# nianticlabs/mickey

Hardware: NVIDIA H100
Metric: image-pairs/sec @720x540 (higher is better)
Workload: dtype f16 operands / f32 accumulate (tensor core), f32 matcher+solver

## Files before the change

include/mickey_b200.h:

```cpp
#ifndef MICKEY_B200_H
#define MICKEY_B200_H

#ifdef __cplusplus
extern "C" {
#endif

typedef struct mk_handle mk_handle;

typedef struct mk_config {
  int embed_dim, depth, heads;
  int down_factor;
  int block_dims[4];
  int desc_dim;
  int use_softmax;
  int depth_sigmoid;
  float max_depth;
  int kp_pos_enc, dsc_pos_enc;
  int norm_dsc;
  float temperature;
  int use_dustbin;
  int it_matches, it_ransac;
  int num_sampled, num_corr, num_refine;
  float th_inlier, th_soft_inlier;
} mk_config;
// ... 111 lines not shown
#define MK_RB_GRAD_W2 4
#define MK_RB_GRAD_WSC 8
#define MK_RB_GRAD_BN1_W 16
#define MK_RB_GRAD_BN1_B 32
#define MK_RB_GRAD_BN2_W 64
#define MK_RB_GRAD_BN2_B 128
typedef struct mk_resblock_params {
  const float* w1; const float* w2; const float* wsc;
  const float* bn1_w; const float* bn1_b; float* bn1_mean; float* bn1_var;
  const float* bn2_w; const float* bn2_b; float* bn2_mean; float* bn2_var;
  float eps1, eps2, momentum1, momentum2;
} mk_resblock_params;
typedef struct mk_resblock_grads {
  float* dx; float* w1; float* w2; float* wsc; float* bn1_w; float* bn1_b; float* bn2_w; float* bn2_b;
} mk_resblock_grads;
long long mk_resblock_ws_bytes(int B, int h, int w, int cin, int cout);
long long mk_resblock_saved_bytes(int B, int h, int w, int cin, int cout);
long long mk_resblock_backward_ws_bytes(int B, int h, int w, int cin, int cout);
int mk_resblock_forward(const float* x_dev, const long long* x_strides_host, int B, int h, int w, int cin, int cout,
                        const mk_resblock_params* params_host, int flags, float* out_dev, void* saved_dev,
                        long long saved_bytes, void* ws_dev, long long ws_bytes, void* stream);
int mk_resblock_backward(const void* saved_dev, const float* grad_out_dev, const long long* g_strides_host,
                         const float* out_dev, int B, int h, int w, int cin, int cout, const mk_resblock_params* params_host,
                         int flags, int want, const mk_resblock_grads* grads_host, void* ws_dev, long long ws_bytes,
                         void* stream);

#define MK_HO_SCORE_SOFTMAX 0
#define MK_HO_SCORE_SIGMOID 1
#define MK_HO_OFFSET 2
#define MK_HO_DEPTH 3
#define MK_HO_DEPTH_SIGMOID 4
#define MK_HO_DESC_L2 5
long long mk_head_out_backward_ws_bytes(int kind, int B, int h, int w, int C);
int mk_head_out_forward(int kind, const float* x_dev, const long long* x_strides_host, int B, int C, int h, int w,
                        const float* weight_dev, const float* eps_dev, float temperature, float max_depth, float* out_dev,
                        float* norm_dev, void* stream);
int mk_head_out_backward(int kind, const float* x_dev, const long long* x_strides_host, int B, int C, int h, int w,
                         const float* weight_dev, float temperature, float max_depth, const float* out_dev,
                         const float* norm_dev, const float* grad_out_dev, float* grad_x_dev, float* grad_w_dev, void* ws_dev,
                         long long ws_bytes, void* stream);

int mk_set_seed(mk_handle* h, unsigned long long seed, void* stream);

long long mk_launch_count(mk_handle* h);
int mk_pdl_enabled(void);
int mk_profile_enable(mk_handle* h, int enable);
int mk_profile_read(mk_handle* h, char* buf, int buf_bytes);

typedef struct mk_gemm_args {
  int epi;
  int impl;
  const void* a; long long a_rows, a_cols, a_ld;
  const void* b; long long b_rows, b_cols, b_ld;
  int M, N, k_chunks, chunks_per_tap, num_taps;
  int tap_shift[9];
  int groups, a_row_group_off, a_col_group_off, a_col_base, b_row_group_off;
  int act;
  const float* bias; int bias_group_off;
  const float* gamma; const float* beta; int ln_group_off;
  float* out_f; long long out_f_ld, out_f_group_off;
  void* out_h; long long out_h_ld, out_h_group_off;
  const void* res_h; long long res_h_ld, res_h_group_off;
  const float* aux; int aux_group_mask;
  int pad_h2, pad_w2, tok_per_img;
  float eps;
  int n_valid; float inv_temp;
  const float* dustbin;
  float* part_row; float* part_col; int part_ld;
  const float* lse_r; const float* lse_c;
  const float* scr0; const float* scr1;
  float* scores; float* kp_scores; float* final_scores;
  float lse_bound;
  long long out_pitch;
} mk_gemm_args;

int mk_op_gemm(const mk_gemm_args* args, void* stream);
int mk_op_patch_gather(const float* img, void* patches_h, int n_img, int H, int W, int kpad, float* x_f,
                       const float* cls_pos, int D, void* stream);
int mk_op_ingest_u8(const unsigned char* img_u8, void* patches_h, int n_img, int H, int W, int kpad, float* x_f,
                    const float* cls_pos, int D, void* stream);
int mk_op_layernorm(const float* x, const float* w, const float* b, void* out_h, int rows, int D, float eps, int mode,
                    int gh, int gw, void* stream);
int mk_op_attention(const void* qkv_h, void* out_h, int n_img, int T, int D, int heads, int impl, void* stream);
int mk_op_linattn(const float* qkv_f, float* kv_part_f, float* kv_f, void* msg_h, int n_img, int G, int h2, int w2, float eps,
                  void* stream);
int mk_op_matcher_reduce(const float* part_row, const float* part_col, const float* dustbin, int B, int N, int part_ld,
                         float* lse_r, float* lse_c, void* stream);
int mk_op_sample(const float* final_scores, int B, int N, long long pitch, int IM, int n_sample, unsigned long long seed, void* ws,
                 long long ws_bytes, int* idx_out, int* status, void* stream);
long long mk_op_sample_workspace_bytes(int B, int IM);
int mk_op_kabsch(const double* H, double* R, int n, void* stream);

int mk_resblock_layout(int B, int h, int w, int cin, int cout, long long* saved_off, long long* bwd_off);
long long mk_op_conv_tf32_ws_bytes(int mode, int B, int h, int w, int cin, int cout, int taps);
int mk_op_conv_tf32(int mode, const float* a, const float* b, float* out, int B, int h, int w, int cin, int cout, int taps,
                    void* ws, long long ws_bytes, void* stream);

#ifdef __cplusplus
}
#endif
#endif
```

mickey_b200/_lib.py:

```python
from __future__ import annotations

import ctypes as C
import math
import os

import torch

_HERE = os.path.dirname(os.path.abspath(__file__))
LIB_PATH = os.path.join(_HERE, "_C", "libmickey_b200.so")


class MkConfig(C.Structure):
    _fields_ = [
        ("embed_dim", C.c_int), ("depth", C.c_int), ("heads", C.c_int),
        ("down_factor", C.c_int),
        ("block_dims", C.c_int * 4),
        ("desc_dim", C.c_int),
        ("use_softmax", C.c_int), ("depth_sigmoid", C.c_int), ("max_depth", C.c_float),
        ("kp_pos_enc", C.c_int), ("dsc_pos_enc", C.c_int), ("norm_dsc", C.c_int),
        ("temperature", C.c_float), ("use_dustbin", C.c_int),
        ("it_matches", C.c_int), ("it_ransac", C.c_int),
        ("num_sampled", C.c_int), ("num_corr", C.c_int), ("num_refine", C.c_int),
        ("th_inlier", C.c_float), ("th_soft_inlier", C.c_float),
    ]
# ... 63 lines not shown
    "mk_extract_images": (C.c_int, [C.c_void_p, C.c_void_p, C.c_int, C.c_int, C.c_int, C.c_void_p, C.c_void_p, C.c_void_p,
                                    C.c_void_p, C.c_void_p, C.c_longlong, C.c_void_p]),
    "mk_extract_images_u8": (C.c_int, [C.c_void_p, C.c_void_p, C.c_int, C.c_int, C.c_int, C.c_void_p, C.c_void_p, C.c_void_p,
                                       C.c_void_p, C.c_void_p, C.c_longlong, C.c_void_p]),
    "mk_forward_pairs": (C.c_int, [C.c_void_p, C.c_void_p, C.c_void_p, C.c_void_p, C.c_void_p, C.c_int,
                                   C.c_void_p, C.c_void_p, C.c_void_p, C.c_void_p, C.c_int,
                                   C.c_void_p, C.c_void_p, C.c_void_p, C.c_void_p, C.c_int, C.c_ulonglong,
                                   C.c_void_p, C.c_void_p, C.c_void_p, C.c_void_p, C.c_void_p, C.c_longlong,
                                   C.c_void_p, C.c_void_p, C.c_void_p, C.c_void_p, C.c_void_p, C.c_void_p, C.c_longlong,
                                   C.c_void_p]),
    "mk_backbone_ws_bytes": (C.c_longlong, [C.c_void_p, C.c_int, C.c_int, C.c_int]),
    "mk_backbone_features": (C.c_int, [C.c_void_p, C.c_void_p, C.c_int, C.c_int, C.c_int, C.c_void_p, C.c_void_p,
                                       C.c_longlong, C.c_void_p]),
    "mk_match": (C.c_int, [C.c_void_p, C.c_int, C.c_void_p, C.c_void_p, C.c_void_p, C.c_longlong, C.c_void_p, C.c_longlong, C.c_void_p]),
    "mk_solve_pose": (C.c_int, [C.c_void_p, C.c_void_p, C.c_longlong, C.c_void_p, C.c_void_p, C.c_void_p, C.c_void_p, C.c_int, C.c_int,
                                C.c_ulonglong, C.c_void_p, C.c_void_p, C.c_void_p, C.c_void_p, C.c_void_p, C.c_void_p,
                                C.c_void_p, C.c_void_p, C.c_void_p, C.c_longlong, C.c_void_p]),
    "mk_forward": (C.c_int, [C.c_void_p, C.c_void_p, C.c_void_p, C.c_void_p, C.c_int, C.c_int, C.c_int, C.c_ulonglong,
                             C.c_void_p, C.c_void_p, C.c_void_p, C.c_void_p, C.c_void_p, C.c_void_p, C.c_void_p, C.c_longlong,
                             C.c_void_p, C.c_void_p, C.c_void_p, C.c_void_p, C.c_void_p, C.c_void_p, C.c_longlong,
                             C.c_void_p]),
    "mk_forward_u8": (C.c_int, [C.c_void_p, C.c_void_p, C.c_void_p, C.c_void_p, C.c_int, C.c_int, C.c_int, C.c_ulonglong,
                                C.c_void_p, C.c_void_p, C.c_void_p, C.c_void_p, C.c_void_p, C.c_void_p, C.c_void_p, C.c_longlong,
                                C.c_void_p, C.c_void_p, C.c_void_p, C.c_void_p, C.c_void_p, C.c_void_p, C.c_longlong,
                                C.c_void_p]),
    "mk_mutual_matches": (C.c_int, [C.c_void_p, C.c_longlong, C.c_int, C.c_int, C.c_float, C.c_void_p, C.c_void_p,
                                    C.c_void_p, C.c_void_p, C.c_longlong, C.c_void_p]),
    "mk_mutual_matches_ws_bytes": (C.c_longlong, [C.c_int, C.c_int]),
    "mk_loss_search": (C.c_int, [C.c_void_p, C.c_longlong, C.c_void_p, C.c_void_p, C.c_void_p, C.c_void_p, C.c_void_p,
                                 C.c_void_p, C.c_int, C.c_int, C.c_int, C.c_int, C.c_int, C.c_int, C.c_int, C.c_float,
                                 C.c_ulonglong, C.c_void_p, C.c_void_p, C.c_void_p, C.c_void_p, C.c_void_p, C.c_void_p,
                                 C.c_void_p, C.c_longlong, C.c_void_p]),
    "mk_loss_search_ws_bytes": (C.c_longlong, [C.c_int, C.c_int]),
    "mk_loss_gradient": (C.c_int, [C.c_void_p, C.c_void_p, C.c_void_p, C.c_void_p, C.c_int, C.c_int, C.c_int, C.c_int,
                                   C.c_void_p, C.c_void_p, C.c_longlong, C.c_void_p]),
    "mk_loss_gradient_ws_bytes": (C.c_longlong, [C.c_int, C.c_int, C.c_int]),
    "mk_dual_softmax_ws_bytes": (C.c_longlong, [C.c_int, C.c_int]),
    "mk_dual_softmax_backward_ws_bytes": (C.c_longlong, [C.c_int, C.c_int]),
    "mk_dual_softmax": (C.c_int, [C.c_void_p, C.c_void_p, C.c_void_p, C.c_void_p, C.c_void_p, C.c_float, C.c_int, C.c_int,
                                  C.c_int, C.c_void_p, C.c_void_p, C.c_void_p, C.c_longlong, C.c_void_p, C.c_void_p,
                                  C.c_void_p, C.c_longlong, C.c_void_p]),
    "mk_dual_softmax_backward": (C.c_int, [C.c_void_p, C.c_void_p, C.c_void_p, C.c_void_p, C.c_void_p, C.c_float, C.c_int,
                                           C.c_int, C.c_void_p, C.c_void_p, C.c_void_p, C.c_longlong, C.c_void_p,
                                           C.c_longlong, C.c_void_p, C.c_longlong, C.c_void_p, C.c_void_p, C.c_void_p,
                                           C.c_void_p, C.c_void_p, C.c_void_p, C.c_longlong, C.c_void_p]),
    "mk_head_transformer_ws_bytes": (C.c_longlong, [C.c_int, C.c_int, C.c_int, C.c_int, C.c_int]),
    "mk_head_transformer_backward_ws_bytes": (C.c_longlong, [C.c_int, C.c_int, C.c_int, C.c_int]),
    "mk_head_transformer": (C.c_int, [C.c_void_p, C.c_void_p, C.c_int, C.c_int, C.c_int, C.POINTER(MkHtrLayer), C.c_int,
                                      C.c_void_p, C.c_int, C.c_void_p, C.c_longlong, C.c_void_p]),
    "mk_head_transformer_backward": (C.c_int, [C.c_void_p, C.c_void_p, C.c_int, C.c_int, C.c_int, C.POINTER(MkHtrLayer),
                                               C.c_int, C.c_void_p, C.POINTER(MkHtrLayerGrads), C.c_void_p, C.c_longlong,
                                               C.c_void_p]),
    "mk_resblock_ws_bytes": (C.c_longlong, [C.c_int, C.c_int, C.c_int, C.c_int, C.c_int]),
    "mk_resblock_saved_bytes": (C.c_longlong, [C.c_int, C.c_int, C.c_int, C.c_int, C.c_int]),
    "mk_resblock_backward_ws_bytes": (C.c_longlong, [C.c_int, C.c_int, C.c_int, C.c_int, C.c_int]),
    "mk_resblock_forward": (C.c_int, [C.c_void_p, C.POINTER(C.c_longlong), C.c_int, C.c_int, C.c_int, C.c_int, C.c_int,
                                      C.POINTER(MkResblockParams), C.c_int, C.c_void_p, C.c_void_p, C.c_longlong,
                                      C.c_void_p, C.c_longlong, C.c_void_p]),
    "mk_resblock_layout": (C.c_int, [C.c_int, C.c_int, C.c_int, C.c_int, C.c_int, C.POINTER(C.c_longlong),
                                     C.POINTER(C.c_longlong)]),
    "mk_resblock_backward": (C.c_int, [C.c_void_p, C.c_void_p, C.POINTER(C.c_longlong), C.c_void_p, C.c_int, C.c_int,
                                       C.c_int, C.c_int, C.c_int, C.POINTER(MkResblockParams), C.c_int, C.c_int,
                                       C.POINTER(MkResblockGrads), C.c_void_p, C.c_longlong, C.c_void_p]),
    "mk_head_out_backward_ws_bytes": (C.c_longlong, [C.c_int, C.c_int, C.c_int, C.c_int, C.c_int]),
    "mk_head_out_forward": (C.c_int, [C.c_int, C.c_void_p, C.POINTER(C.c_longlong), C.c_int, C.c_int, C.c_int, C.c_int,
                                      C.c_void_p, C.c_void_p, C.c_float, C.c_float, C.c_void_p, C.c_void_p, C.c_void_p]),
    "mk_head_out_backward": (C.c_int, [C.c_int, C.c_void_p, C.POINTER(C.c_longlong), C.c_int, C.c_int, C.c_int, C.c_int,
                                       C.c_void_p, C.c_float, C.c_float, C.c_void_p, C.c_void_p, C.c_void_p, C.c_void_p,
                                       C.c_void_p, C.c_void_p, C.c_longlong, C.c_void_p]),
    "mk_pose_to_submission": (C.c_int, [C.c_void_p, C.c_int, C.c_void_p, C.c_void_p]),
    "mk_launch_count": (C.c_longlong, [C.c_void_p]),
    "mk_pdl_enabled": (C.c_int, []),
    "mk_set_seed": (C.c_int, [C.c_void_p, C.c_ulonglong, C.c_void_p]),
    "mk_profile_enable": (C.c_int, [C.c_void_p, C.c_int]),
    "mk_profile_read": (C.c_int, [C.c_void_p, C.c_char_p, C.c_int]),
    "mk_op_gemm": (C.c_int, [C.POINTER(MkGemmArgs), C.c_void_p]),
    "mk_op_patch_gather": (C.c_int, [C.c_void_p, C.c_void_p, C.c_int, C.c_int, C.c_int, C.c_int, C.c_void_p, C.c_void_p,
                                     C.c_int, C.c_void_p]),
    "mk_op_ingest_u8": (C.c_int, [C.c_void_p, C.c_void_p, C.c_int, C.c_int, C.c_int, C.c_int, C.c_void_p, C.c_void_p,
                                  C.c_int, C.c_void_p]),
    "mk_op_layernorm": (C.c_int, [C.c_void_p, C.c_void_p, C.c_void_p, C.c_void_p, C.c_int, C.c_int, C.c_float, C.c_int,
                                  C.c_int, C.c_int, C.c_void_p]),
    "mk_op_attention": (C.c_int, [C.c_void_p, C.c_void_p, C.c_int, C.c_int, C.c_int, C.c_int, C.c_int, C.c_void_p]),
    "mk_op_linattn": (C.c_int, [C.c_void_p, C.c_void_p, C.c_void_p, C.c_void_p, C.c_int, C.c_int, C.c_int, C.c_int, C.c_float, C.c_void_p]),
    "mk_op_matcher_reduce": (C.c_int, [C.c_void_p, C.c_void_p, C.c_void_p, C.c_int, C.c_int, C.c_int, C.c_void_p, C.c_void_p, C.c_void_p]),
    "mk_op_sample": (C.c_int, [C.c_void_p, C.c_int, C.c_int, C.c_longlong, C.c_int, C.c_int, C.c_ulonglong, C.c_void_p, C.c_longlong,
                               C.c_void_p, C.c_void_p, C.c_void_p]),
    "mk_op_sample_workspace_bytes": (C.c_longlong, [C.c_int, C.c_int]),
    "mk_op_kabsch": (C.c_int, [C.c_void_p, C.c_void_p, C.c_int, C.c_void_p]),
    "mk_op_conv_tf32_ws_bytes": (C.c_longlong, [C.c_int, C.c_int, C.c_int, C.c_int, C.c_int, C.c_int, C.c_int]),
    "mk_op_conv_tf32": (C.c_int, [C.c_int, C.c_void_p, C.c_void_p, C.c_void_p, C.c_int, C.c_int, C.c_int, C.c_int, C.c_int,
                                  C.c_int, C.c_void_p, C.c_longlong, C.c_void_p]),
}

STRUCTS = {"mk_config": MkConfig, "mk_gemm_args": MkGemmArgs, "mk_htr_layer": MkHtrLayer,
           "mk_htr_layer_grads": MkHtrLayerGrads, "mk_resblock_params": MkResblockParams,
           "mk_resblock_grads": MkResblockGrads}

_lib = None


class MickeyB200Error(RuntimeError):
    pass


def load():
    global _lib
    if _lib is not None:
        return _lib
    if not os.path.exists(LIB_PATH):
        raise MickeyB200Error(
            f"{LIB_PATH} not found. Build it with `python -m mickey_b200.build` (needs nvcc; sm_90a only). "
            "mickey_b200 has no CPU or PyTorch fallback.")
    lib = C.CDLL(LIB_PATH)
    for name, (res, args) in EXPORTS.items():
        fn = getattr(lib, name)
        fn.restype = res
        fn.argtypes = args
    sizes = {name: (lib.mk_sizeof(name.encode()), C.sizeof(st)) for name, st in STRUCTS.items()}
    bad = [f"{name} {lib_size} vs {py_size}" for name, (lib_size, py_size) in sizes.items() if lib_size != py_size]
    if bad:
        raise MickeyB200Error("ctypes struct layout does not match the library (stale build?): " + ", ".join(bad))
    _lib = lib
    return lib


def check(rc: int, what: str = ""):
    if rc != 0:
        msg = load().mk_last_error().decode(errors="replace")
        raise MickeyB200Error(f"{what} failed (code {rc}): {msg}")


def ptr(t):
    return None if t is None else C.c_void_p(t.data_ptr())


def stream(dev=None):
    return C.c_void_p(torch.cuda.current_stream(dev).cuda_stream)


def workspace(nbytes, dev, what: str):
    nbytes = int(nbytes)
    if nbytes < 0:
        raise MickeyB200Error(f"{what} returned {nbytes}: {load().mk_last_error().decode(errors='replace')}")
    return torch.empty(max(nbytes, 1), dtype=torch.uint8, device=dev)


def pitched(t):
    B, N, _ = t.shape
    s0, s1, s2 = t.stride()
    if s2 == 1 and s1 >= N and (B == 1 or s0 == N * s1):
        return t, s1
    return t.contiguous(), N


class Handle:

    def __init__(self, device, cfg: MkConfig):
        self.lib = load()
        self.device = device
        h = C.c_void_p()
        check(self.lib.mk_create(device.index or 0, C.byref(cfg), C.byref(h)), "mk_create")
        self.h = h

    def __del__(self):
        try:
# ... 17 lines not shown
```

mickey_b200/csrc/attention_tc.cu:

```cuda
#include "gemm_tc.cuh"
#include "ops.h"
#include "gemm.h"
#include <algorithm>
#include <cstdlib>
#include <cstring>

namespace mk {

constexpr int FA_BQ = 192, FA_BK = 128, FA_D = 64, FA_KV_STAGES = 4;
constexpr int FA_CONSUMERS = 3, FA_THREADS = 128 * (FA_CONSUMERS + 1), FA_WARP_TMA = 4 * FA_CONSUMERS;
constexpr int FA_REGS_PRODUCER = 32, FA_REGS_CONSUMER = 160;
static_assert(FA_REGS_PRODUCER * 128 + FA_REGS_CONSUMER * 128 * FA_CONSUMERS <= 65536, "attention: register budget");
constexpr int FA_Q_BYTES = FA_BQ * 128;
constexpr int FA_KV_BYTES = FA_BK * 128;
constexpr int FA_O_BYTES = 64 * 128;
constexpr int FA_REGION = 2 * FA_Q_BYTES + 2 * FA_KV_STAGES * FA_KV_BYTES + FA_CONSUMERS * FA_O_BYTES;
constexpr int FA_SMEM = FA_REGION + 1024 + 256;
static_assert(FA_SMEM <= 227 * 1024, "attention: shared memory");

__device__ __forceinline__ float ex2_approx(float x) {
  float y;
  asm("ex2.approx.ftz.f32 %0, %1;" : "=f"(y) : "f"(x));
  return y;
}

__device__ __forceinline__ void wgmma_m64n64k16_rs_tb(float (&d)[32], const uint32_t (&a)[4], uint64_t desc_b) {
  asm volatile(
      "{\n\t.reg .pred p;\n\tsetp.ne.b32 p, %37, 0;\n\t"
      "wgmma.mma_async.sync.aligned.m64n64k16.f32.f16.f16 "
      "{%0, %1, %2, %3, %4, %5, %6, %7, %8, %9, %10, %11, %12, %13, %14, %15, %16, %17, %18, %19, %20, %21, %22, %23, %24, %25, %26, %27, %28, %29, %30, %31}, {%32, %33, %34, %35}, %36, p, 1, 1, 1;\n\t}"
      : "+f"(d[0]), "+f"(d[1]), "+f"(d[2]), "+f"(d[3]), "+f"(d[4]), "+f"(d[5]), "+f"(d[6]), "+f"(d[7]), "+f"(d[8]), "+f"(d[9]), "+f"(d[10]), "+f"(d[11]), "+f"(d[12]), "+f"(d[13]), "+f"(d[14]), "+f"(d[15]), "+f"(d[16]), "+f"(d[17]), "+f"(d[18]), "+f"(d[19]), "+f"(d[20]), "+f"(d[21]), "+f"(d[22]), "+f"(d[23]), "+f"(d[24]), "+f"(d[25]), "+f"(d[26]), "+f"(d[27]), "+f"(d[28]), "+f"(d[29]), "+f"(d[30]), "+f"(d[31])
      : "r"(a[0]), "r"(a[1]), "r"(a[2]), "r"(a[3]), "l"(desc_b), "r"(1u));
}

__device__ __forceinline__ void warpgroup_sync(int wg) { asm volatile("bar.sync %0, 128;" ::"r"(2 + wg) : "memory"); }

struct AttnTile { int qt, head, im; };
__device__ __forceinline__ AttnTile attn_tile(int t, int q_tiles, int heads) {
  const int bh = t / q_tiles;
  return {t - bh * q_tiles, bh % heads, bh / heads};
}

__device__ __forceinline__ void softmax_tile(float (&s)[64], uint32_t (&p)[8][4], float (&m_run)[2], float (&l_run)[2],
                                             float (&alpha)[2], float scale_log2, int valid, int lane) {
  if (valid < FA_BK) {
#pragma unroll
    for (int i = 0; i < 64; ++i) {
      const int col = 8 * (i >> 2) + 2 * (lane & 3) + (i & 1);
      if (col >= valid) s[i] = -INFINITY;
    }
  }
#pragma unroll
  for (int h = 0; h < 2; ++h) {
    float mx = -INFINITY;
#pragma unroll
    for (int c = 0; c < 16; ++c) mx = fmaxf(mx, fmaxf(s[4 * c + 2 * h], s[4 * c + 2 * h + 1]));
    mx = fmaxf(mx, __shfl_xor_sync(0xffffffffu, mx, 1));
    mx = fmaxf(mx, __shfl_xor_sync(0xffffffffu, mx, 2));
    const float m_new = fmaxf(m_run[h], mx * scale_log2);
    alpha[h] = ex2_approx(m_run[h] - m_new);
    m_run[h] = m_new;
    float sum = 0.f;
#pragma unroll
    for (int c = 0; c < 16; ++c) {
      const float p0 = ex2_approx(fmaf(s[4 * c + 2 * h], scale_log2, -m_new));
      const float p1 = ex2_approx(fmaf(s[4 * c + 2 * h + 1], scale_log2, -m_new));
      const __half2 ph = __floats2half2_rn(p0, p1);
      const float2 r = __half22float2(ph);
      p[c >> 1][2 * (c & 1) + h] = *reinterpret_cast<const uint32_t*>(&ph);
      sum += r.x + r.y;
    }
    l_run[h] = l_run[h] * alpha[h] + sum;
  }
}

__global__ void __launch_bounds__(FA_THREADS, 1)
attention_tc_kernel(const __grid_constant__ CUtensorMap tmQ, const __grid_constant__ CUtensorMap tmKV,
                    const __grid_constant__ CUtensorMap tmO, int T, int heads, int q_tiles, int n_tiles_total, float scale_log2) {
  extern __shared__ uint8_t smem_raw[];
  const uint32_t raw = smem_u32(smem_raw);
  const uint32_t base = (raw + 1023u) & ~1023u;
  const uint32_t sQ = base;
  const uint32_t sK = sQ + 2 * FA_Q_BYTES;
  const uint32_t sV = sK + FA_KV_STAGES * FA_KV_BYTES;
  const uint32_t sO = sV + FA_KV_STAGES * FA_KV_BYTES;
  const uint32_t bars = base + FA_REGION;
  const uint32_t k_full = bars, k_empty = k_full + 8 * FA_KV_STAGES, v_full = k_empty + 8 * FA_KV_STAGES,
                 v_empty = v_full + 8 * FA_KV_STAGES, q_full = v_empty + 8 * FA_KV_STAGES, q_empty = q_full + 16;

  const int warp = threadIdx.x >> 5, lane = threadIdx.x & 31;
  const int D = heads * FA_D;
  const int n_kv = (T + FA_BK - 1) / FA_BK;

  if (warp == FA_WARP_TMA && lane == 0) {
    asm volatile("prefetch.tensormap [%0];" ::"l"(&tmQ) : "memory");
    asm volatile("prefetch.tensormap [%0];" ::"l"(&tmKV) : "memory");
    asm volatile("prefetch.tensormap [%0];" ::"l"(&tmO) : "memory");
    for (int s = 0; s < FA_KV_STAGES; ++s) {
      mbar_init(k_full + 8 * s, 1); mbar_init(k_empty + 8 * s, 4 * FA_CONSUMERS);
      mbar_init(v_full + 8 * s, 1); mbar_init(v_empty + 8 * s, 4 * FA_CONSUMERS);
    }
    for (int b = 0; b < 2; ++b) { mbar_init(q_full + 8 * b, 1); mbar_init(q_empty + 8 * b, 4 * FA_CONSUMERS); }
    asm volatile("fence.mbarrier_init.release.cluster;" ::: "memory");
  }
  __syncthreads();
  pdl_wait();

  if (warp >= FA_WARP_TMA) {
    setmaxnreg_dec<FA_REGS_PRODUCER>();
    if (warp == FA_WARP_TMA && elect_one()) {
      int st = 0;
      uint32_t ph = 0;
      int it = 0;
      for (int t = blockIdx.x; t < n_tiles_total; t += gridDim.x, ++it) {
        const AttnTile tile = attn_tile(t, q_tiles, heads);
        const int row_base = tile.im * T;
        const int qb = it & 1;
        mbar_wait(q_empty + 8 * qb, ((it >> 1) & 1) ^ 1);
        mbar_expect_tx(q_full + 8 * qb, FA_Q_BYTES);
        tma_load_2d(sQ + qb * FA_Q_BYTES, &tmQ, q_full + 8 * qb, tile.head * FA_D, row_base + tile.qt * FA_BQ);
        for (int j = 0; j < n_kv; ++j) {
          mbar_wait(k_empty + 8 * st, ph ^ 1);
          mbar_expect_tx(k_full + 8 * st, FA_KV_BYTES);
          tma_load_2d(sK + st * FA_KV_BYTES, &tmKV, k_full + 8 * st, D + tile.head * FA_D, row_base + j * FA_BK);
          mbar_wait(v_empty + 8 * st, ph ^ 1);
          mbar_expect_tx(v_full + 8 * st, FA_KV_BYTES);
          tma_load_2d(sV + st * FA_KV_BYTES, &tmKV, v_full + 8 * st, 2 * D + tile.head * FA_D, row_base + j * FA_BK);
          if (++st == FA_KV_STAGES) { st = 0; ph ^= 1; }
        }
      }
    }
    __syncwarp();
    pdl_trigger();
    return;
  }

  setmaxnreg_inc<FA_REGS_CONSUMER>();
  const int wg = warp >> 2;
  const uint32_t stage_o = sO + wg * FA_O_BYTES;
  int ks = 0, vs = 0;
  uint32_t kph = 0, vph = 0;
  int it = 0;
  for (int t = blockIdx.x; t < n_tiles_total; t += gridDim.x, ++it) {
    const AttnTile tile = attn_tile(t, q_tiles, heads);
    const int qb = it & 1;
    const uint64_t dq = gmma_desc_sw128(sQ + qb * FA_Q_BYTES + wg * (64 * 128));
    float s[64], o[32];
    uint32_t p[8][4];
#pragma unroll
    for (int i = 0; i < 32; ++i) o[i] = 0.f;
    float m_run[2] = {-INFINITY, -INFINITY}, l_run[2] = {0.f, 0.f}, alpha[2];
    mbar_wait(q_full + 8 * qb, (it >> 1) & 1);

    for (int j = 0; j < n_kv; ++j) {
      mbar_wait(k_full + 8 * ks, kph);
      const uint64_t dk = gmma_desc_sw128(sK + ks * FA_KV_BYTES);
      wgmma_fence();
#pragma unroll
      for (int k = 0; k < FA_D / WGMMA_K; ++k) wgmma_m64n128k16(s, dq + (uint64_t)(k * 2), dk + (uint64_t)(k * 2), k > 0 ? 1u : 0u);
      wgmma_commit();
      wgmma_wait<0>();
      reg_fence(s);
      if (lane == 0) mbar_arrive(k_empty + 8 * ks);
      if (++ks == FA_KV_STAGES) { ks = 0; kph ^= 1; }
      softmax_tile(s, p, m_run, l_run, alpha, scale_log2, T - j * FA_BK, lane);
#pragma unroll
      for (int c = 0; c < 8; ++c) {
        o[4 * c] *= alpha[0]; o[4 * c + 1] *= alpha[0];
        o[4 * c + 2] *= alpha[1]; o[4 * c + 3] *= alpha[1];
      }
      mbar_wait(v_full + 8 * vs, vph);
      const uint64_t dv = gmma_desc_sw128(sV + vs * FA_KV_BYTES);
      wgmma_fence();
#pragma unroll
      for (int kk = 0; kk < FA_BK / WGMMA_K; ++kk)
        wgmma_m64n64k16_rs_tb(o, p[kk], dv + (uint64_t)(kk * 128));
      wgmma_commit();
      wgmma_wait<0>();
      reg_fence(o);
      if (lane == 0) mbar_arrive(v_empty + 8 * vs);
      if (++vs == FA_KV_STAGES) { vs = 0; vph ^= 1; }
    }
    if (lane == 0) mbar_arrive(q_empty + 8 * qb);
    if (t + (int)gridDim.x >= n_tiles_total) pdl_trigger();

    const int row0 = tile.qt * FA_BQ + wg * 64;
    if (row0 >= T) continue;
    if (threadIdx.x % 128 == 0) tma_store_wait_read();
    warpgroup_sync(wg);
#pragma unroll
    for (int h = 0; h < 2; ++h) {
      float l = l_run[h];
      l += __shfl_xor_sync(0xffffffffu, l, 1);
      l += __shfl_xor_sync(0xffffffffu, l, 2);
      const float inv = 1.0f / l;
      const int r = (warp & 3) * 16 + (lane >> 2) + 8 * h;
#pragma unroll
      for (int c = 0; c < 8; ++c) {
        const __half2 v = __floats2half2_rn(o[4 * c + 2 * h] * inv, o[4 * c + 2 * h + 1] * inv);
        asm volatile("st.shared.b32 [%0], %1;" ::"r"(stage_o + r * 128 + ((c ^ (r & 7)) << 4) + 4 * (lane & 3)),
                     "r"(*reinterpret_cast<const uint32_t*>(&v)) : "memory");
      }
    }
    fence_async_smem();
    warpgroup_sync(wg);
    if (threadIdx.x % 128 == 0) {
      tma_store_3d(&tmO, stage_o, tile.head * FA_D, row0, tile.im);
      tma_store_commit();
    }
  }
  if (threadIdx.x % 128 == 0) tma_store_wait_all();
}

int attention_tc(const void* qkv, void* out, int n_img, int T, int D, int heads, cudaStream_t s) {
  if (D != heads * FA_D) { set_last_error("attention: head_dim must be 64 (D=%d heads=%d)", D, heads); return MK_ERR_UNSUPPORTED; }
  static unsigned long long attr_mask = 0;
  if (first_use_on_device(attr_mask)) {
    MK_CUDA_CHECK(cudaFuncSetAttribute(attention_tc_kernel, cudaFuncAttributeMaxDynamicSharedMemorySize, FA_SMEM));
  }
  CUtensorMap tmQ, tmKV, tmO;
  int rc = make_tensor_map_f16(&tmQ, qkv, (long long)n_img * T, 3LL * D, 3LL * D, FA_BQ);
  if (!rc) rc = make_tensor_map_f16(&tmKV, qkv, (long long)n_img * T, 3LL * D, 3LL * D, FA_BK);
  if (!rc) rc = make_tensor_map_out_f16(&tmO, out, n_img, T, D, 64);
  if (rc) return rc;
  const int q_tiles = ceil_div(T, FA_BQ);
  const int tiles = q_tiles * heads * n_img;
  const float scale_log2 = 0.125f * 1.4426950408889634f;
  MK_CUDA_CHECK(launch_k(attention_tc_kernel, dim3(std::min(tiles, sm_count())), dim3(FA_THREADS), (size_t)FA_SMEM, s, tmQ, tmKV, tmO,
                         T, heads, q_tiles, tiles, scale_log2));
  return MK_OK;
}

int attention_dispatch(const void* qkv, void* out, int n_img, int T, int D, int heads, int impl, cudaStream_t s) {
  if (impl == 0) {
    static int def = 0;
    if (!def) { const char* e = getenv("MICKEY_ATTN_IMPL"); def = (e && strcmp(e, "mma") == 0) ? 2 : 1; }
    impl = def;
  }
  if (impl != 1 && impl != 2) { set_last_error("attention: unknown impl %d", impl); return MK_ERR_INVALID; }
  return impl == 2 ? attention(qkv, out, n_img, T, D, heads, s) : attention_tc(qkv, out, n_img, T, D, heads, s);
}

}
```

mickey_b200/csrc/engine.cu:

```cuda
#include "../../include/mickey_b200.h"
#include "gemm.h"
#include "ops.h"

#include <algorithm>
#include <cstring>
#include <string>
#include <unordered_map>
#include <vector>

using namespace mk;

struct Tensor { const void* ptr; int dtype; long long numel; };

struct mk_handle {
  int device;
  mk_config cfg;
  std::unordered_map<std::string, Tensor> tensors;
  int geo_h = 0, geo_w = 0;
  bool finalized = false;
  unsigned long long* seed_dev = nullptr;
  long long launches = 0;
  bool profiling = false;
  struct ProfRec { std::string tag; cudaEvent_t e0, e1; };
  std::vector<ProfRec> prof;
// ... 665 lines not shown
  Workspace w = carve(base, h->cfg, g);
  const std::unordered_map<std::string, const void*> m = {
      {"P", w.P}, {"X", w.X}, {"XN", w.XN}, {"QKV", w.QKV}, {"ATT", w.ATT}, {"H1", w.H1}, {"F", w.F}, {"T1", w.T1},
      {"S1", w.S1}, {"O1", w.O1}, {"T2", w.T2}, {"S2", w.S2}, {"O2", w.O2}, {"T3", w.T3}, {"S3", w.S3}, {"CAT", w.CAT},
      {"MSG", w.MSG}, {"HM", w.HM}, {"T4k", w.T4k}, {"S4k", w.S4k}, {"T4d", w.T4d}, {"X32", w.X32}, {"QKV32", w.QKV32},
      {"KV", w.KV}, {"Y4k", w.Y4k}, {"Y4d", w.Y4d}, {"score_raw", w.score_raw}, {"DSCX", w.DSCX}, {"nrm2", w.nrm2},
      {"lse_r", w.lse_r}, {"lse_c", w.lse_c}, {"idx", w.idx}, {"hyp_scores", w.hyp_scores},
      {"hyp_Rt", w.hyp_Rt}};
  auto it = m.find(name);
  if (it == m.end()) { set_last_error("unknown workspace buffer '%s'", name); return -1; }
  return (long long)(reinterpret_cast<const uint8_t*>(it->second) - base);
}

int mk_profile_enable(mk_handle* h, int enable) {
  if (!h) return MK_ERR_INVALID;
  for (auto& r : h->prof) { cudaEventDestroy(r.e0); cudaEventDestroy(r.e1); }
  h->prof.clear();
  h->profiling = enable != 0;
  return MK_OK;
}

int mk_profile_read(mk_handle* h, char* buf, int buf_bytes) {
  if (!h || !buf || buf_bytes <= 0) return MK_ERR_INVALID;
  MK_CUDA_CHECK(cudaDeviceSynchronize());
  std::vector<std::string> order;
  std::unordered_map<std::string, std::pair<int, double>> acc;
  for (auto& r : h->prof) {
    float ms = 0.f;
    if (cudaEventElapsedTime(&ms, r.e0, r.e1) != cudaSuccess) continue;
    if (!acc.count(r.tag)) order.push_back(r.tag);
    acc[r.tag].first += 1;
    acc[r.tag].second += ms;
  }
  std::string out;
  char line[256];
  for (auto& t : order) {
    snprintf(line, sizeof(line), "%s %d %.6f\n", t.c_str(), acc[t].first, acc[t].second);
    out += line;
  }
  if ((int)out.size() + 1 > buf_bytes) { set_last_error("profile buffer too small"); return MK_ERR_INVALID; }
  memcpy(buf, out.c_str(), out.size() + 1);
  return MK_OK;
}

int mk_op_gemm(const mk_gemm_args* a, void* stream) {
  if (!a) return MK_ERR_INVALID;
  GemmParams p;
  memset(&p, 0, sizeof(p));
  p.M = a->M; p.N = a->N; p.k_chunks = a->k_chunks; p.chunks_per_tap = a->chunks_per_tap; p.num_taps = a->num_taps;
  for (int i = 0; i < 9; ++i) p.tap_shift[i] = a->tap_shift[i];
  p.groups = a->groups; p.a_row_group_off = a->a_row_group_off; p.a_col_group_off = a->a_col_group_off;
  p.a_col_base = a->a_col_base; p.b_row_group_off = a->b_row_group_off; p.act = a->act;
  p.bias = a->bias; p.bias_group_off = a->bias_group_off; p.gamma = a->gamma; p.beta = a->beta; p.ln_group_off = a->ln_group_off;
  p.out_f = a->out_f; p.out_f_ld = a->out_f_ld; p.out_f_group_off = a->out_f_group_off;
  p.out_h = (__half*)a->out_h; p.out_h_ld = a->out_h_ld; p.out_h_group_off = a->out_h_group_off;
  p.res_h = (const __half*)a->res_h; p.res_h_ld = a->res_h_ld; p.res_h_group_off = a->res_h_group_off;
  p.aux = a->aux; p.aux_group_mask = a->aux_group_mask; p.pad_h2 = a->pad_h2; p.pad_w2 = a->pad_w2; p.tok_per_img = a->tok_per_img;
  p.eps = a->eps; p.n_valid = a->n_valid; p.inv_temp = a->inv_temp; p.dustbin = a->dustbin;
  p.part_row = reinterpret_cast<float2*>(a->part_row); p.part_col = reinterpret_cast<float2*>(a->part_col); p.part_ld = a->part_ld;
  p.lse_r = a->lse_r; p.lse_c = a->lse_c; p.scr0 = a->scr0; p.scr1 = a->scr1; p.lse_bound = a->lse_bound;
  p.out_pitch = a->out_pitch > 0 ? a->out_pitch : a->n_valid;
  p.out_tma = (a->final_scores && p.out_pitch % 4 == 0 && reinterpret_cast<uintptr_t>(a->final_scores) % 16 == 0 &&
               (!a->scores || (reinterpret_cast<uintptr_t>(a->scores) % 16 == 0 && reinterpret_cast<uintptr_t>(a->kp_scores) % 16 == 0))) ? 1 : 0;
  p.scores = a->scores; p.kp_scores = a->kp_scores; p.final_scores = a->final_scores;
  GemmOperand A{a->a, a->a_rows, a->a_cols, a->a_ld}, B{a->b, a->b_rows, a->b_cols, a->b_ld};
  return launch_gemm(a->epi, A, B, p, (cudaStream_t)stream, a->impl);
}

int mk_op_patch_gather(const float* img, void* P, int n_img, int H, int W, int kpad, float* X, const float* cls_pos,
                       int D, void* stream) {
  return patch_gather(img, P, n_img, H, W, kpad, X, cls_pos, D, (cudaStream_t)stream);
}
int mk_op_ingest_u8(const unsigned char* img, void* P, int n_img, int H, int W, int kpad, float* X, const float* cls_pos,
                    int D, void* stream) {
  return ingest_u8(img, P, n_img, H, W, kpad, X, cls_pos, D, (cudaStream_t)stream);
}
int mk_op_layernorm(const float* x, const float* w, const float* b, void* out, int rows, int D, float eps, int mode,
                    int gh, int gw, void* stream) {
  return layernorm(x, w, b, out, rows, D, eps, mode, gh, gw, (cudaStream_t)stream);
}
int mk_op_attention(const void* qkv, void* out, int n_img, int T, int D, int heads, int impl, void* stream) {
  return attention_dispatch(qkv, out, n_img, T, D, heads, impl, (cudaStream_t)stream);
}
int mk_op_linattn(const float* qkv, float* kv_part, float* kv, void* msg, int n_img, int Gn, int h2, int w2, float eps,
                  void* stream) {
  MK_TRY(linattn_kv(qkv, kv_part, kv, n_img, Gn, h2, w2, (cudaStream_t)stream));
  return linattn_msg(qkv, kv, msg, n_img, Gn, h2, w2, eps, (cudaStream_t)stream);
}
int mk_op_matcher_reduce(const float* part_row, const float* part_col, const float* dustbin, int B, int N, int part_ld,
                         float* lse_r, float* lse_c, void* stream) {
  return matcher_lse_reduce(part_row, part_col, dustbin, B, N, part_ld, lse_r, lse_c, (cudaStream_t)stream);
}
long long mk_op_sample_workspace_bytes(int B, int IM) { return (long long)sampler_workspace_bytes(B, IM) + 512; }
int mk_op_sample(const float* fs, int B, int N, long long pitch, int IM, int n_sample, unsigned long long seed, void* ws,
                 long long ws_bytes, int* idx_out, int* status, void* stream) {
  MK_TRY(resolve_pitch(pitch, N, "mk_op_sample: pitch"));
  if ((long long)sampler_workspace_bytes(B, IM) + 256 > ws_bytes) { set_last_error("sampler workspace too small"); return MK_ERR_INVALID; }
  MK_CUDA_CHECK(cudaMemsetAsync(status, 0, sizeof(int), (cudaStream_t)stream));
  const size_t off = ((size_t)sampler_workspace_bytes(B, IM) + 255) & ~(size_t)255;
  unsigned long long* sd = reinterpret_cast<unsigned long long*>(reinterpret_cast<uint8_t*>(ws) + off);
  MK_TRY(seed_set(sd, seed, (cudaStream_t)stream));
  return sample_outer(fs, B, N, pitch, IM, n_sample, sd, ws, idx_out, status, (cudaStream_t)stream);
}
int mk_op_kabsch(const double* H, double* R, int n, void* stream) { return kabsch_batch(H, R, n, (cudaStream_t)stream); }

}
```

mickey_b200/csrc/ops.h:

```cpp
#pragma once
#include "common.cuh"

namespace mk {

int patch_gather(const float* img, void* P, int n_img, int H, int W, int kpad, float* X, const float* cls_pos, int D, cudaStream_t s);
int layernorm(const float* x, const float* w, const float* b, void* out, int rows, int D, float eps, int mode, int gh, int gw, cudaStream_t s);
int layernorm_channel_major(const float* x, const float* w, const float* b, float* out, int n_img, int N, int D, float eps,
                            cudaStream_t s);
int attention(const void* qkv, void* out, int n_img, int T, int D, int heads, cudaStream_t s);
int attention_tc(const void* qkv, void* out, int n_img, int T, int D, int heads, cudaStream_t s);
int attention_dispatch(const void* qkv, void* out, int n_img, int T, int D, int heads, int impl, cudaStream_t s);

int ingest_u8(const uint8_t* img, void* P, int n_img, int H, int W, int kpad, float* X, const float* cls_pos, int D, cudaStream_t s);
int pose_to_submission(const float* pose, int n, double* out, cudaStream_t s);

int linattn_kv_chunks(int h2, int w2);
int linattn_kv(const float* qkv, float* kv_part, float* kv, int n_img, int G, int h2, int w2, cudaStream_t s);
int linattn_msg(const float* qkv, const float* kv, void* msg, int n_img, int G, int h2, int w2, float eps, cudaStream_t s);
int kp_head_out(const float* y, const float* w_depth, const float* w_xy, const float* w_score, float* depth, float* kps,
                float* score_raw, float* scr, int n_img, int gh, int gw, int depth_sigmoid, float max_depth,
                float down_factor, int use_softmax, cudaStream_t s);
int desc_out(const float* y, float* dsc_cm, void* dsc_x, float* nrm2, int n_img, int gh, int gw, int normalize, cudaStream_t s);
int matcher_lse_reduce(const void* part_row, const void* part_col, const float* dustbin, int B, int N, int part_ld, float* lse_r,
                       float* lse_c, cudaStream_t s);
struct BankView { const float *kps, *depth, *scr, *dsc; const int* idx; int count; };
int bank_gather(const BankView& b0, const BankView& b1, int P, int N, void* dsc_x, float* kps_out, float* depth_out, float* scr_out,
                cudaStream_t s);
int bank_index_check(const BankView& b0, const BankView& b1, int P, float* pose, int* status, cudaStream_t s);

long long mutual_matches_ws_bytes(int B, int N);
int mutual_matches(const float* scores, long long pitch, int B, int N, float min_conf, int* matches, float* match_scores,
                   int* count, void* ws, long long ws_bytes, cudaStream_t s);

struct RansacParams {
  int it_matches, it_ransac, n_sample, n_corr, n_refine;
  float th_inlier, th_soft;
  const unsigned long long* seed;
};
int seed_set(unsigned long long* s, unsigned long long v, cudaStream_t st);
int seed_advance(unsigned long long* s, cudaStream_t st);
size_t sampler_workspace_bytes(int B, int IM);
int sample_outer(const float* final_scores, int B, int N, long long pitch, int IM, int n_sample, const unsigned long long* seed,
                 void* ws, int* idx_out, int* status, cudaStream_t st, int invalid_bits = 1);
int ransac_solve(const float* final_scores, long long pitch, const float* kps0, const float* d0, const float* kps1, const float* d1,
                 const float* K0, const float* K1, int B, int N, const RansacParams& rp, const int* outer_idx,
                 const int* inner_idx, float* hyp_scores, float* hyp_Rt, int* counters, float* pose,
                 int* best_set, float* inl_mask, int* best_hyp, cudaStream_t st);
int kabsch_batch(const double* H, double* R, int n, cudaStream_t st);
constexpr int SOLVER_COUNTER_BASE = 4;

constexpr int LOSS_MAX_C = 16, LOSS_MAX_S = 2048;
long long loss_search_ws_bytes(int B, int IM);
int loss_search(const float* fs, long long pitch, const float* kps0, const float* d0, const float* kps1, const float* d1,
                const float* K0, const float* K1, int B, int N, int IM, int IR, int S, int C, int n_ref, float th_ref,
                unsigned long long seed, const int* outer_idx, const int* inner_idx, int* sampled_out, int* inner_out,
                uint32_t* inl_out, int* status, void* ws, long long ws_bytes, cudaStream_t st);
long long loss_gradient_ws_bytes(int B, int IM, int S);
int loss_gradient(const int* sampled, const float* loss_value, const float* baseline, const float* mask, int B, int N, int IM,
                  int S, float* grad, void* ws, long long ws_bytes, cudaStream_t st);

}
```

Measured before the change: 308.1.

## Ping-pong warpgroup scheduling and QK/PV overlap in TMA attention kernel

Adds a scheduled variant of the Hopper flash-attention kernel, now the default impl. A named-barrier ring serialises WGMMA issue across the three consumer warpgroups, and each warpgroup issues the next tile's QK product together with the current PV product, so softmax in one warpgroup overlaps tensor-core work in another. It also specialises softmax for masked and unmasked tiles, skips compute on dead query rows, and rotates the starting q-tile per head to spread tail work. A trace entry point with clock64 stamps is added for profiling; the extra barrier ring and the larger register live ranges from holding s and o together could add stalls or spills.

```diff
diff --git a/include/mickey_b200.h b/include/mickey_b200.h
--- a/include/mickey_b200.h
+++ b/include/mickey_b200.h
@@ -217,6 +217,8 @@
 int mk_op_layernorm(const float* x, const float* w, const float* b, void* out_h, int rows, int D, float eps, int mode,
                     int gh, int gw, void* stream);
 int mk_op_attention(const void* qkv_h, void* out_h, int n_img, int T, int D, int heads, int impl, void* stream);
+int mk_op_attention_trace(const void* qkv_h, void* out_h, int n_img, int T, int D, int heads, int sched, long long* trace,
+                          void* stream);
 int mk_op_linattn(const float* qkv_f, float* kv_part_f, float* kv_f, void* msg_h, int n_img, int G, int h2, int w2, float eps,
                   void* stream);
 int mk_op_matcher_reduce(const float* part_row, const float* part_col, const float* dustbin, int B, int N, int part_ld,
diff --git a/mickey_b200/_lib.py b/mickey_b200/_lib.py
--- a/mickey_b200/_lib.py
+++ b/mickey_b200/_lib.py
@@ -169,6 +169,8 @@
     "mk_op_layernorm": (C.c_int, [C.c_void_p, C.c_void_p, C.c_void_p, C.c_void_p, C.c_int, C.c_int, C.c_float, C.c_int,
                                   C.c_int, C.c_int, C.c_void_p]),
     "mk_op_attention": (C.c_int, [C.c_void_p, C.c_void_p, C.c_int, C.c_int, C.c_int, C.c_int, C.c_int, C.c_void_p]),
+    "mk_op_attention_trace": (C.c_int, [C.c_void_p, C.c_void_p, C.c_int, C.c_int, C.c_int, C.c_int, C.c_int, C.c_void_p,
+                                        C.c_void_p]),
     "mk_op_linattn": (C.c_int, [C.c_void_p, C.c_void_p, C.c_void_p, C.c_void_p, C.c_int, C.c_int, C.c_int, C.c_int, C.c_float, C.c_void_p]),
     "mk_op_matcher_reduce": (C.c_int, [C.c_void_p, C.c_void_p, C.c_void_p, C.c_int, C.c_int, C.c_int, C.c_void_p, C.c_void_p, C.c_void_p]),
     "mk_op_sample": (C.c_int, [C.c_void_p, C.c_int, C.c_int, C.c_longlong, C.c_int, C.c_int, C.c_ulonglong, C.c_void_p, C.c_longlong,
diff --git a/mickey_b200/csrc/attention_tc.cu b/mickey_b200/csrc/attention_tc.cu
--- a/mickey_b200/csrc/attention_tc.cu
+++ b/mickey_b200/csrc/attention_tc.cu
@@ -38,12 +38,16 @@
 struct AttnTile { int qt, head, im; };
 __device__ __forceinline__ AttnTile attn_tile(int t, int q_tiles, int heads) {
   const int bh = t / q_tiles;
-  return {t - bh * q_tiles, bh % heads, bh / heads};
-}
-
+  int qt = t - bh * q_tiles + bh % q_tiles;
+  if (qt >= q_tiles) qt -= q_tiles;
+  return {qt, bh % heads, bh / heads};
+}
+
+template <bool MASKED>
 __device__ __forceinline__ void softmax_tile(float (&s)[64], uint32_t (&p)[8][4], float (&m_run)[2], float (&l_run)[2],
                                              float (&alpha)[2], float scale_log2, int valid, int lane) {
-  if (valid < FA_BK) {
+  const int blocks = MASKED ? (valid + 7) >> 3 : 16;
+  if (MASKED) {
 #pragma unroll
     for (int i = 0; i < 64; ++i) {
       const int col = 8 * (i >> 2) + 2 * (lane & 3) + (i & 1);
@@ -54,7 +58,8 @@
   for (int h = 0; h < 2; ++h) {
     float mx = -INFINITY;
 #pragma unroll
-    for (int c = 0; c < 16; ++c) mx = fmaxf(mx, fmaxf(s[4 * c + 2 * h], s[4 * c + 2 * h + 1]));
+    for (int c = 0; c < 16; ++c)
+      if (!MASKED || c < blocks) mx = fmaxf(mx, fmaxf(s[4 * c + 2 * h], s[4 * c + 2 * h + 1]));
     mx = fmaxf(mx, __shfl_xor_sync(0xffffffffu, mx, 1));
     mx = fmaxf(mx, __shfl_xor_sync(0xffffffffu, mx, 2));
     const float m_new = fmaxf(m_run[h], mx * scale_log2);
@@ -63,6 +68,7 @@
     float sum = 0.f;
 #pragma unroll
     for (int c = 0; c < 16; ++c) {
+      if (MASKED && c >= blocks) { p[c >> 1][2 * (c & 1) + h] = 0u; continue; }
       const float p0 = ex2_approx(fmaf(s[4 * c + 2 * h], scale_log2, -m_new));
       const float p1 = ex2_approx(fmaf(s[4 * c + 2 * h + 1], scale_log2, -m_new));
       const __half2 ph = __floats2half2_rn(p0, p1);
@@ -74,9 +80,40 @@
   }
 }
 
+__device__ __forceinline__ void softmax_step(float (&s)[64], uint32_t (&p)[8][4], float (&m_run)[2], float (&l_run)[2],
+                                             float (&alpha)[2], float scale_log2, int valid, int lane) {
+  if (valid < FA_BK) softmax_tile<true>(s, p, m_run, l_run, alpha, scale_log2, valid, lane);
+  else softmax_tile<false>(s, p, m_run, l_run, alpha, scale_log2, valid, lane);
+}
+
+__device__ __forceinline__ void qk_batch(float (&s)[64], uint64_t dq, uint64_t dk) {
+#pragma unroll
+  for (int k = 0; k < FA_D / WGMMA_K; ++k) wgmma_m64n128k16(s, dq + (uint64_t)(k * 2), dk + (uint64_t)(k * 2), k > 0 ? 1u : 0u);
+}
+
+__device__ __forceinline__ void pv_batch(float (&o)[32], const uint32_t (&p)[8][4], uint64_t dv) {
+#pragma unroll
+  for (int kk = 0; kk < FA_BK / WGMMA_K; ++kk) wgmma_m64n64k16_rs_tb(o, p[kk], dv + (uint64_t)(kk * 128));
+}
+
+__device__ __forceinline__ void rescale(float (&o)[32], const float (&alpha)[2]) {
+#pragma unroll
+  for (int c = 0; c < 8; ++c) {
+    o[4 * c] *= alpha[0]; o[4 * c + 1] *= alpha[0];
+    o[4 * c + 2] *= alpha[1]; o[4 * c + 3] *= alpha[1];
+  }
+}
+
+__device__ __forceinline__ void ring_take(int wg) { asm volatile("bar.sync %0, 256;" ::"r"(5 + wg) : "memory"); }
+__device__ __forceinline__ void ring_pass(int wg) { asm volatile("bar.arrive %0, 256;" ::"r"(5 + (wg == 2 ? 0 : wg + 1)) : "memory"); }
+
+enum { TR_QK_ISSUED, TR_QK_RETIRED, TR_SOFTMAX_DONE, TR_PV_ISSUED, TR_PV_RETIRED, FA_TRACE_POINTS };
+
+template <bool SCHED, bool TRACE>
 __global__ void __launch_bounds__(FA_THREADS, 1)
 attention_tc_kernel(const __grid_constant__ CUtensorMap tmQ, const __grid_constant__ CUtensorMap tmKV,
-                    const __grid_constant__ CUtensorMap tmO, int T, int heads, int q_tiles, int n_tiles_total, float scale_log2) {
+                    const __grid_constant__ CUtensorMap tmO, int T, int heads, int q_tiles, int n_tiles_total, float scale_log2,
+                    long long* trace) {
   extern __shared__ uint8_t smem_raw[];
   const uint32_t raw = smem_u32(smem_raw);
   const uint32_t base = (raw + 1023u) & ~1023u;
@@ -141,51 +178,111 @@
   int ks = 0, vs = 0;
   uint32_t kph = 0, vph = 0;
   int it = 0;
+  if (SCHED && wg == 2) ring_pass(2);
   for (int t = blockIdx.x; t < n_tiles_total; t += gridDim.x, ++it) {
     const AttnTile tile = attn_tile(t, q_tiles, heads);
     const int qb = it & 1;
     const uint64_t dq = gmma_desc_sw128(sQ + qb * FA_Q_BYTES + wg * (64 * 128));
+    long long* tr = nullptr;
+    if (TRACE && blockIdx.x == 0 && it < 2 && lane == 0 && warp % 4 == 0) tr = trace + (long long)(it * 3 + wg) * n_kv * FA_TRACE_POINTS;
+    const auto stamp = [&](int j, int point) { if (TRACE && tr) tr[j * FA_TRACE_POINTS + point] = clock64(); };
     float s[64], o[32];
     uint32_t p[8][4];
 #pragma unroll
     for (int i = 0; i < 32; ++i) o[i] = 0.f;
     float m_run[2] = {-INFINITY, -INFINITY}, l_run[2] = {0.f, 0.f}, alpha[2];
     mbar_wait(q_full + 8 * qb, (it >> 1) & 1);
-
-    for (int j = 0; j < n_kv; ++j) {
+    const bool live = tile.qt * FA_BQ + wg * 64 < T;
+
+    if (!live) {
+      for (int j = 0; j < n_kv; ++j) {
+        mbar_wait(k_full + 8 * ks, kph);
+        if (SCHED) { ring_take(wg); ring_pass(wg); }
+        stamp(j, TR_QK_ISSUED); stamp(j, TR_QK_RETIRED); stamp(j, TR_SOFTMAX_DONE);
+        if (lane == 0) mbar_arrive(k_empty + 8 * ks);
+        if (++ks == FA_KV_STAGES) { ks = 0; kph ^= 1; }
+        mbar_wait(v_full + 8 * vs, vph);
+        stamp(j, TR_PV_ISSUED); stamp(j, TR_PV_RETIRED);
+        if (lane == 0) mbar_arrive(v_empty + 8 * vs);
+        if (++vs == FA_KV_STAGES) { vs = 0; vph ^= 1; }
+      }
+      if (SCHED) { ring_take(wg); ring_pass(wg); }
+    } else if constexpr (SCHED) {
       mbar_wait(k_full + 8 * ks, kph);
-      const uint64_t dk = gmma_desc_sw128(sK + ks * FA_KV_BYTES);
+      ring_take(wg);
       wgmma_fence();
-#pragma unroll
-      for (int k = 0; k < FA_D / WGMMA_K; ++k) wgmma_m64n128k16(s, dq + (uint64_t)(k * 2), dk + (uint64_t)(k * 2), k > 0 ? 1u : 0u);
+      qk_batch(s, dq, gmma_desc_sw128(sK + ks * FA_KV_BYTES));
       wgmma_commit();
+      ring_pass(wg);
+      stamp(0, TR_QK_ISSUED);
       wgmma_wait<0>();
       reg_fence(s);
+      stamp(0, TR_QK_RETIRED);
       if (lane == 0) mbar_arrive(k_empty + 8 * ks);
       if (++ks == FA_KV_STAGES) { ks = 0; kph ^= 1; }
-      softmax_tile(s, p, m_run, l_run, alpha, scale_log2, T - j * FA_BK, lane);
-#pragma unroll
-      for (int c = 0; c < 8; ++c) {
-        o[4 * c] *= alpha[0]; o[4 * c + 1] *= alpha[0];
-        o[4 * c + 2] *= alpha[1]; o[4 * c + 3] *= alpha[1];
-      }
-      mbar_wait(v_full + 8 * vs, vph);
-      const uint64_t dv = gmma_desc_sw128(sV + vs * FA_KV_BYTES);
-      wgmma_fence();
-#pragma unroll
-      for (int kk = 0; kk < FA_BK / WGMMA_K; ++kk)
-        wgmma_m64n64k16_rs_tb(o, p[kk], dv + (uint64_t)(kk * 128));
-      wgmma_commit();
-      wgmma_wait<0>();
-      reg_fence(o);
-      if (lane == 0) mbar_arrive(v_empty + 8 * vs);
-      if (++vs == FA_KV_STAGES) { vs = 0; vph ^= 1; }
+      for (int j = 0; j < n_kv; ++j) {
+        softmax_step(s, p, m_run, l_run, alpha, scale_log2, T - j * FA_BK, lane);
+        rescale(o, alpha);
+        stamp(j, TR_SOFTMAX_DONE);
+        const bool next = j + 1 < n_kv;
+        mbar_wait(v_full + 8 * vs, vph);
+        if (next) mbar_wait(k_full + 8 * ks, kph);
+        const uint64_t dv = gmma_desc_sw128(sV + vs * FA_KV_BYTES), dk = gmma_desc_sw128(sK + ks * FA_KV_BYTES);
+        ring_take(wg);
+        wgmma_fence();
+        pv_batch(o, p, dv);
+        if (next) {
+          wgmma_fence();
+          qk_batch(s, dq, dk);
+        }
+        wgmma_commit();
+        ring_pass(wg);
+        stamp(j, TR_PV_ISSUED);
+        if (next) stamp(j + 1, TR_QK_ISSUED);
+        wgmma_wait<0>();
+        reg_fence(o);
+        reg_fence(s);
+        stamp(j, TR_PV_RETIRED);
+        if (next) stamp(j + 1, TR_QK_RETIRED);
+        if (lane == 0) mbar_arrive(v_empty + 8 * vs);
+        if (++vs == FA_KV_STAGES) { vs = 0; vph ^= 1; }
+        if (next) {
+          if (lane == 0) mbar_arrive(k_empty + 8 * ks);
+          if (++ks == FA_KV_STAGES) { ks = 0; kph ^= 1; }
+        }
+      }
+    } else {
+      for (int j = 0; j < n_kv; ++j) {
+        mbar_wait(k_full + 8 * ks, kph);
+        wgmma_fence();
+        qk_batch(s, dq, gmma_desc_sw128(sK + ks * FA_KV_BYTES));
+        wgmma_commit();
+        stamp(j, TR_QK_ISSUED);
+        wgmma_wait<0>();
+        reg_fence(s);
+        stamp(j, TR_QK_RETIRED);
+        if (lane == 0) mbar_arrive(k_empty + 8 * ks);
+        if (++ks == FA_KV_STAGES) { ks = 0; kph ^= 1; }
+        softmax_step(s, p, m_run, l_run, alpha, scale_log2, T - j * FA_BK, lane);
+        rescale(o, alpha);
+        stamp(j, TR_SOFTMAX_DONE);
+        mbar_wait(v_full + 8 * vs, vph);
+        wgmma_fence();
+        pv_batch(o, p, gmma_desc_sw128(sV + vs * FA_KV_BYTES));
+        wgmma_commit();
+        stamp(j, TR_PV_ISSUED);
+        wgmma_wait<0>();
+        reg_fence(o);
+        stamp(j, TR_PV_RETIRED);
+        if (lane == 0) mbar_arrive(v_empty + 8 * vs);
+        if (++vs == FA_KV_STAGES) { vs = 0; vph ^= 1; }
+      }
     }
     if (lane == 0) mbar_arrive(q_empty + 8 * qb);
     if (t + (int)gridDim.x >= n_tiles_total) pdl_trigger();
 
+    if (!live) continue;
     const int row0 = tile.qt * FA_BQ + wg * 64;
-    if (row0 >= T) continue;
     if (threadIdx.x % 128 == 0) tma_store_wait_read();
     warpgroup_sync(wg);
 #pragma unroll
@@ -209,14 +306,16 @@
       tma_store_commit();
     }
   }
+  if (SCHED && wg == 0) ring_take(0);
   if (threadIdx.x % 128 == 0) tma_store_wait_all();
 }
 
-int attention_tc(const void* qkv, void* out, int n_img, int T, int D, int heads, cudaStream_t s) {
+template <bool SCHED, bool TRACE>
+static int attention_tc(const void* qkv, void* out, int n_img, int T, int D, int heads, long long* trace, cudaStream_t s) {
   if (D != heads * FA_D) { set_last_error("attention: head_dim must be 64 (D=%d heads=%d)", D, heads); return MK_ERR_UNSUPPORTED; }
   static unsigned long long attr_mask = 0;
   if (first_use_on_device(attr_mask)) {
-    MK_CUDA_CHECK(cudaFuncSetAttribute(attention_tc_kernel, cudaFuncAttributeMaxDynamicSharedMemorySize, FA_SMEM));
+    MK_CUDA_CHECK(cudaFuncSetAttribute(attention_tc_kernel<SCHED, TRACE>, cudaFuncAttributeMaxDynamicSharedMemorySize, FA_SMEM));
   }
   CUtensorMap tmQ, tmKV, tmO;
   int rc = make_tensor_map_f16(&tmQ, qkv, (long long)n_img * T, 3LL * D, 3LL * D, FA_BQ);
@@ -226,9 +325,15 @@
   const int q_tiles = ceil_div(T, FA_BQ);
   const int tiles = q_tiles * heads * n_img;
   const float scale_log2 = 0.125f * 1.4426950408889634f;
-  MK_CUDA_CHECK(launch_k(attention_tc_kernel, dim3(std::min(tiles, sm_count())), dim3(FA_THREADS), (size_t)FA_SMEM, s, tmQ, tmKV, tmO,
-                         T, heads, q_tiles, tiles, scale_log2));
+  MK_CUDA_CHECK(launch_k(attention_tc_kernel<SCHED, TRACE>, dim3(std::min(tiles, sm_count())), dim3(FA_THREADS), (size_t)FA_SMEM, s,
+                         tmQ, tmKV, tmO, T, heads, q_tiles, tiles, scale_log2, trace));
   return MK_OK;
+}
+
+int attention_trace(const void* qkv, void* out, int n_img, int T, int D, int heads, int sched, long long* trace, cudaStream_t s) {
+  if (!trace) { set_last_error("attention_trace: null trace buffer"); return MK_ERR_INVALID; }
+  return sched ? attention_tc<true, true>(qkv, out, n_img, T, D, heads, trace, s)
+               : attention_tc<false, true>(qkv, out, n_img, T, D, heads, trace, s);
 }
 
 int attention_dispatch(const void* qkv, void* out, int n_img, int T, int D, int heads, int impl, cudaStream_t s) {
@@ -237,8 +342,12 @@
     if (!def) { const char* e = getenv("MICKEY_ATTN_IMPL"); def = (e && strcmp(e, "mma") == 0) ? 2 : 1; }
     impl = def;
   }
-  if (impl != 1 && impl != 2) { set_last_error("attention: unknown impl %d", impl); return MK_ERR_INVALID; }
-  return impl == 2 ? attention(qkv, out, n_img, T, D, heads, s) : attention_tc(qkv, out, n_img, T, D, heads, s);
-}
-
-}
+  switch (impl) {
+    case 1: return attention_tc<true, false>(qkv, out, n_img, T, D, heads, nullptr, s);
+    case 2: return attention(qkv, out, n_img, T, D, heads, s);
+    case 3: return attention_tc<false, false>(qkv, out, n_img, T, D, heads, nullptr, s);
+    default: set_last_error("attention: unknown impl %d", impl); return MK_ERR_INVALID;
+  }
+}
+
+}
diff --git a/mickey_b200/csrc/engine.cu b/mickey_b200/csrc/engine.cu
--- a/mickey_b200/csrc/engine.cu
+++ b/mickey_b200/csrc/engine.cu
@@ -771,6 +771,9 @@
 int mk_op_attention(const void* qkv, void* out, int n_img, int T, int D, int heads, int impl, void* stream) {
   return attention_dispatch(qkv, out, n_img, T, D, heads, impl, (cudaStream_t)stream);
 }
+int mk_op_attention_trace(const void* qkv, void* out, int n_img, int T, int D, int heads, int sched, long long* trace, void* stream) {
+  return attention_trace(qkv, out, n_img, T, D, heads, sched, trace, (cudaStream_t)stream);
+}
 int mk_op_linattn(const float* qkv, float* kv_part, float* kv, void* msg, int n_img, int Gn, int h2, int w2, float eps,
                   void* stream) {
   MK_TRY(linattn_kv(qkv, kv_part, kv, n_img, Gn, h2, w2, (cudaStream_t)stream));
diff --git a/mickey_b200/csrc/ops.h b/mickey_b200/csrc/ops.h
--- a/mickey_b200/csrc/ops.h
+++ b/mickey_b200/csrc/ops.h
@@ -8,8 +8,8 @@
 int layernorm_channel_major(const float* x, const float* w, const float* b, float* out, int n_img, int N, int D, float eps,
                             cudaStream_t s);
 int attention(const void* qkv, void* out, int n_img, int T, int D, int heads, cudaStream_t s);
-int attention_tc(const void* qkv, void* out, int n_img, int T, int D, int heads, cudaStream_t s);
 int attention_dispatch(const void* qkv, void* out, int n_img, int T, int D, int heads, int impl, cudaStream_t s);
+int attention_trace(const void* qkv, void* out, int n_img, int T, int D, int heads, int sched, long long* trace, cudaStream_t s);
 
 int ingest_u8(const uint8_t* img, void* P, int n_img, int H, int W, int kpad, float* X, const float* cls_pos, int D, cudaStream_t s);
 int pose_to_submission(const float* pose, int n, double* out, cudaStream_t s);
```

After: 313.0, median of 6. 1.02x the previous value.
